# secup/ProjectUltra

Hardware: AMD Instinct MI355X
Metric: OFDM-1024 16QAM R3/4 frames decoded/sec (higher is better)
Workload: dtype f32

## Files before the change

### projectultra_amd/csrc/demod_kernel.h

```cpp
#ifndef ULTRA_DEMOD_KERNEL_H
#define ULTRA_DEMOD_KERNEL_H

#include <hip/hip_runtime.h>
#include <utility>
#include "device_types.h"
#include "pinned_math.h"
#include "phase_table.h"

namespace ultra_hip {
namespace dev {

constexpr int kWave = 64;
constexpr int kPhaseCap = 48;

__device__ __forceinline__ c32 mk(float re, float im) { c32 r; r.re = re; r.im = im; return r; }
__device__ __forceinline__ c32 cadd(c32 a, c32 b) { return mk(a.re + b.re, a.im + b.im); }
__device__ __forceinline__ c32 csub(c32 a, c32 b) { return mk(a.re - b.re, a.im - b.im); }
__device__ __forceinline__ c32 cconj(c32 a) { return mk(a.re, -a.im); }
__device__ __forceinline__ c32 cmul(c32 x, c32 y) {
    float ac = x.re * y.re, bd = x.im * y.im, ad = x.re * y.im, bc = x.im * y.re;
    return mk(ac - bd, ad + bc);
}
__device__ __forceinline__ c32 cdiv(c32 x, c32 y) {
    double a = x.re, b = x.im, c = y.re, d = y.im;
// ... 857 lines not shown
                        const float dist = dr * dr + di * di;
                        if (bits & mask) { if (dist < m1) m1 = dist; }
                        else { if (dist < m0) m0 = dist; }
                    }
                }
                out[b] = clip_llr(sf * (m1 - m0));
            }
            break;
        }
        case ULTRA_MOD_QAM64: {
            const float I = sym.re, Q = sym.im, scale = 2.0f / nv;
            const float D2 = 0.3086067f, D4 = 0.6172134f;
            out[0] = clip_llr(-scale * I);
            out[1] = clip_llr(scale * (fabsf(I) - D4));
            out[2] = clip_llr(scale * (fabsf(fabsf(I) - D4) - D2));
            out[3] = clip_llr(-scale * Q);
            out[4] = clip_llr(scale * (fabsf(Q) - D4));
            out[5] = clip_llr(scale * (fabsf(fabsf(Q) - D4) - D2));
            break;
        }
        case ULTRA_MOD_QAM256: {
            const float I = sym.re, Q = sym.im, scale = 2.0f / nv;
            const float D2 = 0.1290994f, D4 = 0.2581989f, D8 = 0.5163978f;
            out[0] = clip_llr(-scale * I);
            out[1] = clip_llr(scale * (fabsf(I) - D8));
            out[2] = clip_llr(scale * (fabsf(fabsf(I) - D8) - D4));
            out[3] = clip_llr(scale * (fabsf(fabsf(fabsf(I) - D8) - D4) - D2));
            out[4] = clip_llr(-scale * Q);
            out[5] = clip_llr(scale * (fabsf(Q) - D8));
            out[6] = clip_llr(scale * (fabsf(fabsf(Q) - D8) - D4));
            out[7] = clip_llr(scale * (fabsf(fabsf(fabsf(Q) - D8) - D4) - D2));
            break;
        }
        case ULTRA_MOD_QPSK:
        default: {
            const float scale = (-2.0f * 0.7071067811865476f) / nv;
            out[0] = clip_llr(sym.re * scale);
            out[1] = clip_llr(sym.im * scale);
            break;
        }
    }
}

__device__ __forceinline__ float slice8(float x, float d) {
    if (x < -6 * d) return -7 * d;
    if (x < -4 * d) return -5 * d;
    if (x < -2 * d) return -3 * d;
    if (x < 0) return -d;
    if (x < 2 * d) return d;
    if (x < 4 * d) return 3 * d;
    if (x < 6 * d) return 5 * d;
    return 7 * d;
}
template <int MOD>
__device__ __forceinline__ c32 hard_decision(c32 sym) {
    if (MOD == ULTRA_MOD_BPSK) return mk(sym.re > 0 ? 1.0f : -1.0f, 0.0f);
    if (MOD == ULTRA_MOD_QAM16) {
        auto slice = [](float x) { return (x < -0.4f) ? -0.9487f : (x < 0.0f) ? -0.3162f : (x < 0.4f) ? 0.3162f : 0.9487f; };
        return mk(slice(sym.re), slice(sym.im));
    }
    if (MOD == ULTRA_MOD_QAM32) {
        const float d = 0.1961161351381840f;
        const float I = (sym.re < -2 * d) ? -3 * d : (sym.re < 0) ? -d : (sym.re < 2 * d) ? d : 3 * d;
        return mk(I, slice8(sym.im, d));
    }
    if (MOD == ULTRA_MOD_QAM64) return mk(slice8(sym.re, 0.1543f), slice8(sym.im, 0.1543f));
    return mk(sym.re > 0 ? 0.7071f : -0.7071f, sym.im > 0 ? 0.7071f : -0.7071f);
}
struct AdaptiveEq { c32 w; float P; };

template <int MOD>
__device__ __forceinline__ void equalize_demap(TrackShared& sh, const DemodConst& D, const LaneConst& lc, Track& tr,
                                               c32& dprev, const c32* __restrict__ fq, float* __restrict__ llr_sym,
                                               float* dprev_abs = nullptr, const c32* tc_fixed = nullptr,
                                               const c32* received_in = nullptr, AdaptiveEq* ad = nullptr, c32* eq_out = nullptr) {
    constexpr bool kDiff = (MOD == ULTRA_MOD_DBPSK || MOD == ULTRA_MOD_DQPSK || MOD == ULTRA_MOD_D8PSK);
    constexpr int kBits = (MOD == ULTRA_MOD_DBPSK || MOD == ULTRA_MOD_BPSK) ? 1 : (MOD == ULTRA_MOD_DQPSK || MOD == ULTRA_MOD_QPSK) ? 2
                        : (MOD == ULTRA_MOD_D8PSK) ? 3 : (MOD == ULTRA_MOD_QAM16) ? 4 : (MOD == ULTRA_MOD_QAM32) ? 5
                        : (MOD == ULTRA_MOD_QAM64) ? 6 : 8;
    const int lane = threadIdx.x;
    const int nd = D.n_data;
    const bool is_data = lane < nd;
    c32 eq = mk(0.0f, 0.0f);
    float nv = 100.0f;
    if (kDiff) {
        if (is_data) {
            const c32 received = fq[lc.data_fq], h = sh.H[lc.data_slot];
            const float h_power = cnorm(h);
            const c32 tc = tc_fixed ? *tc_fixed : cexpj_bounded(timing_phase_of(lc.data_k, tr.timing, D.log2_fft));
            if (h_power > 1e-6f) {
                const c32 t = cdivf(cmul(received, cconj(h)), h_power);
                eq = cmul(cmul(t, tr.ppc), tc);
                nv = tr.noise_variance / h_power;
            } else {
                eq = cmul(cmul(received, tr.ppc), tc);
                nv = 100.0f;
            }
            nv = fmax_std(1e-6f, fmin_std(100.0f, nv));
        }
    } else {
        float h_power = 0.0f;
        if (is_data) {
            const c32 received = received_in ? *received_in : fq[lc.data_fq], h = sh.H[lc.data_slot];
            h_power = cnorm(h);
            if (ad) {
                const c32 w = ad->w;
                const float w_power = cnorm(w), denom = w_power + tr.noise_variance;
                if (denom < 1e-10f) {
                    eq = mk(0.0f, 0.0f);
                    nv = 100.0f;
                } else {
                    eq = cdivf(cmul(cconj(w), received), denom);
                    nv = tr.noise_variance / (w_power + 1e-6f);
                }
                if (D.decision_directed) {
                    const c32 ref = hard_decision<MOD>(eq);
                    const c32 err = csub(received, cmul(w, ref));
                    if (D.adaptive_eq == 2) {
                        const float lambda = D.rls_lambda, P = ad->P, ref_norm = cnorm(ref);
                        const float k = P / (lambda + P * ref_norm);
                        ad->w = cadd(w, cmul(cscale(cconj(ref), k), err));
                        const float Pn = (P - k * ref_norm * P) / lambda;
                        ad->P = fmax_std(0.001f, fmin_std(1000.0f, Pn));
                    } else {
                        ad->w = cadd(w, cmul(cscale(cconj(ref), D.lms_mu), err));
                    }
                }
            } else {
            const float mmse_denom = h_power + tr.noise_variance;
            if (mmse_denom < 1e-10f) {
                eq = mk(0.0f, 0.0f);
                nv = 100.0f;
            } else {
                eq = cdivf(cmul(cconj(h), received), mmse_denom);
                nv = tr.noise_variance / (h_power + 1e-6f);
                nv = fmax_std(1e-6f, fmin_std(100.0f, nv));
            }
            }
        }
        const float T = wave_sum_unordered(is_data ? h_power : 0.0f);
        const float thr = T * D.fade_k, lo = thr * 0.99993896484375f, hi = thr * 1.00006103515625f;
        const bool t_plain = T >= 0x1p-60f && T <= 0x1p60f;
        const bool close = is_data && !(h_power < lo) && !(h_power >= hi);
        if (__builtin_expect(t_plain && !__any(close), 1)) {
            if (is_data && h_power < lo) nv = 100.0f;
        } else {
            float avg = ordered_sum(sh.fbuf, h_power, nd);
            avg /= (float)nd;
            if (is_data && h_power < 0.1f * avg) nv = 100.0f;
        }
    }

    if (eq_out && is_data) eq_out[lane] = eq;
    if (kDiff && !tr.has_dprev) { dprev = mk(1.0f, 0.0f); if (dprev_abs) *dprev_abs = -1.0f; }
    float eq_abs = -1.0f;
    if (is_data) {
        if (kDiff) {
            eq_abs = cabs_(eq);
            const float pa = (dprev_abs && *dprev_abs >= 0.0f) ? *dprev_abs : cabs_(dprev);
            demap_carrier<MOD>(eq, dprev, nv * D.ce_margin, llr_sym + lane * kBits, eq_abs, pa);
            dprev = eq;
            if (dprev_abs) *dprev_abs = eq_abs;
        } else {
            demap_carrier<MOD>(eq, dprev, nv * D.ce_margin, llr_sym + lane * kBits);
        }
    }
    if ((MOD == ULTRA_MOD_DQPSK || MOD == ULTRA_MOD_D8PSK) && tr.snr_symbol_count >= 1) {
        bool strong = false;
        if (is_data) {
            const float a = eq_abs;
            strong = (a * a) > 0.1f;
            if (strong) sh.H[lc.data_slot] = cmul(sh.H[lc.data_slot], mk(1.0f, -0.0f));
        }
        const int valid = __popcll(__ballot(strong));
        if (valid >= 5) {
            c32 p = cmul(cscale(tr.ppc, 1.0f), mk(1.0f, -0.0f));
            const float mag = cabs_(p);
            if (mag > 0.01f) p = cdivf(p, mag);
            tr.ppc = p;
        }
    }
    if (kDiff) tr.has_dprev = 1;
    wave_sync();
}

__device__ __forceinline__ void lts_symbol(TrackShared& sh, const DemodConst& D, const LaneConst& lc, int sym,
                                           int n_train, c32& lts_acc, const c32* __restrict__ fq) {
    const int lane = threadIdx.x;
    if (lane < D.n_data && sym == n_train - 1) {
        c32 h = mk(0.0f, 0.0f);
        if (cabs_(lc.zc) > 0.01f) h = cdiv(fq[lc.data_fq], lc.zc);
        sh.H[lc.data_slot] = h;
    }
    if (lane < D.n_pilot) {
        if (sym == 0) lts_acc = mk(0.0f, 0.0f);
        if (cabs_(lc.pilot_seq) > 0.01f) lts_acc = cadd(lts_acc, cdiv_pilot(fq[lc.pilot_fq], lc.pilot_seq));
    }
    wave_sync();
}

__device__ __forceinline__ void lts_finish(TrackShared& sh, const DemodConst& D, const LaneConst& lc, Track& tr,
                                           int n_train, c32 lts_acc) {
    const int lane = threadIdx.x;
    const float inv_count = 1.0f / (float)n_train;
    if (lane < D.n_pilot) sh.H[lc.pilot_slot] = cscale(lts_acc, inv_count);
    wave_sync();
    float mag = 0.0f;
    if (lane < D.n_data) mag = cabs_(sh.H[lc.data_slot]);
    const float h_mag_avg = ordered_sum(sh.fbuf, mag, D.n_data) / (float)D.n_data;
    if (h_mag_avg > 1e-6f && tr.noise_variance > 1e-10f) {
        const float s = (h_mag_avg * h_mag_avg) / tr.noise_variance;
        tr.snr_linear = fmax_std(0.1f, fmin_std(10000.0f, s));
    }
    tr.snr_symbol_count = n_train;
    wave_sync();
}


__global__ __launch_bounds__(kWave) void init_state_kernel(const float* __restrict__ cfo_hz,
                                                           const float* __restrict__ cfo_phase, int n_frames,
                                                           float* __restrict__ state, int compact, int adaptive,
                                                           const float* __restrict__ timing = nullptr) {
    const int lane = threadIdx.x;
    for (int frame = blockIdx.x; frame < n_frames; frame += gridDim.x) {
        float* st = state + (size_t)frame * kStFloats;
        if (adaptive) {
            reinterpret_cast<c32*>(st + kStLms)[lane] = mk(1.0f, 0.0f);
            st[kStRlsP + lane] = 1.0f;
        }
        if (!compact) reinterpret_cast<c32*>(st + kStH)[lane] = mk(1.0f, 0.0f);
        if (lane < 32) reinterpret_cast<c32*>(st + kStHp)[lane] = mk(1.0f, 0.0f);
        if (lane < 16) {
            float v = 0.0f;
            const float cfo = cfo_hz ? cfo_hz[frame] : 0.0f;
            if (lane == st_cfo || lane == st_cfo_filt) v = cfo;
            else if (lane == st_cfo_phase) v = cfo_phase ? cfo_phase[frame] : 0.0f;
            else if (lane == st_noise) v = 0.1f;
            else if (lane == st_snr) v = 1.0f;
            else if (lane == st_timing) v = timing ? timing[frame] : 0.0f;
            else if (lane == st_ppc_re || lane == st_cpc_re) v = 1.0f;
            st[lane] = v;
        }
    }
}

__global__ __launch_bounds__(kWave) void resync_state_kernel(const float* __restrict__ cfo_hz, const float* __restrict__ cfo_phase,
                                                             int n_frames, float* __restrict__ state, int reset_carrier_phase) {
    const int lane = threadIdx.x;
    for (int frame = blockIdx.x; frame < n_frames; frame += gridDim.x) {
        float* st = state + (size_t)frame * kStFloats;
        if (lane < 16) {
            float v = st[lane];
            const float cfo = cfo_hz ? cfo_hz[frame] : 0.0f;
            if (lane == st_cfo || lane == st_cfo_filt) v = cfo;
            else if (lane == st_cfo_phase) v = cfo_phase ? cfo_phase[frame] : 0.0f;
            else if (lane == st_timing || lane == st_since) v = 0.0f;
            else if (lane == st_flags) {
                int flags = (int)v & ~4;
                if (reset_carrier_phase) flags &= ~1;
                v = (float)flags;
            } else if (reset_carrier_phase && lane == st_cpc_re) v = 1.0f;
            else if (reset_carrier_phase && lane == st_cpc_im) v = 0.0f;
            st[lane] = v;
        }
    }
}

__global__ __launch_bounds__(256) void train_cfo_kernel(const DemodConst* __restrict__ Dp, const c32* __restrict__ nco,
                                                        const float* __restrict__ audio, size_t frame_stride,
                                                        const unsigned* __restrict__ frame_offset, const float* __restrict__ cfo_in,
                                                        int n_frames, float* __restrict__ state) {
    const DemodConst& D = *Dp;
    const int frame = blockIdx.x * blockDim.x + threadIdx.x;
    if (frame >= n_frames || !cfo_in) return;
    const float given = cfo_in[frame];
    if (given == given) return;
    float* st = state + (size_t)frame * kStFloats;
    float cfo = 0.0f;
    if (D.n_train >= 2) {
        const float* x = audio + (size_t)frame * frame_stride + (frame_offset ? frame_offset[frame] : 0u);
        const int N = D.fft, cp = D.cp, S = D.sym_len;
        c32 P = mk(0.0f, 0.0f);
        float E1 = 0.0f, E2 = 0.0f;
        for (int i = 0; i < N; ++i) {
            const c32 o1 = nco[cp + i], o2 = nco[S + cp + i];
            const float a1 = x[cp + i], a2 = x[S + cp + i];
            const c32 z1 = mk(a1 * o1.re, a1 * -o1.im), z2 = mk(a2 * o2.re, a2 * -o2.im);
            const c32 pr = cmul(mk(z1.re, -z1.im), z2);
            P = mk(P.re + pr.re, P.im + pr.im);
            E1 += z1.re * z1.re + z1.im * z1.im;
            E2 += z2.re * z2.re + z2.im * z2.im;
        }
        const float corr = um::hypotf_(P.re, P.im) / sqrtf(E1 * E2 + 1e-10f);
        if (!(corr < 0.3f)) {
            const float phase = um::atan2f_(P.im, P.re);
            cfo = (float)((double)(phase * D.sample_rate) / ((double)2.0f * 3.14159265358979323846 * (double)S));
            const float max_cfo = D.sample_rate / (2.0f * (float)S);
            cfo = fmaxf(-max_cfo, fminf(max_cfo, cfo));
        }
    }
    st[st_cfo] = cfo; st[st_cfo_filt] = cfo; st[st_cfo_phase] = 0.0f;
}

__device__ __forceinline__ float walk_to_table(const DemodConst& D, float cfo, float phase, unsigned* __restrict__ tab) {
    tab[3] = __float_as_uint(phase);
    tab[1] = __float_as_uint(cfo);
    if (!(fabsf(cfo) > 0.01f)) { tab[0] = 0u; tab[2] = __float_as_uint(phase); return phase; }
    const float inc = (float)(((-kTwoPi) * (double)cfo) / (double)D.sample_rate);
    int covered;
    float pnext;
    const int ns = um::phase_table_walk(phase, inc, D.sym_len, kPhaseCap, &covered, &pnext,
                                        [&](int k, int start, float base, float step) {
                                            tab[4 + 3 * k] = (unsigned)start;
                                            tab[5 + 3 * k] = __float_as_uint(base);
                                            tab[6 + 3 * k] = __float_as_uint(step);
                                        });
    const unsigned bounded = (fabsf(phase) <= 4.0f && fabsf(inc) <= 1.0f) ? 0x80000000u : 0u;
    tab[0] = (unsigned)ns | ((unsigned)covered << 8) | bounded; tab[2] = __float_as_uint(pnext);
    for (int done = covered; done < D.sym_len;) {
        int c2;
        float p2;
        um::phase_table_walk(pnext, inc, D.sym_len - done, kPhaseCap, &c2, &p2, [](int, int, float, float) {});
        done += c2;
        pnext = p2;
    }
    return pnext;
}

__global__ __launch_bounds__(256) void cfo_walk_kernel(const DemodConst* __restrict__ Dp, int n_frames,
                                                       float* __restrict__ state, unsigned* __restrict__ seg_tab) {
    const DemodConst& D = *Dp;
    const int frame = blockIdx.x * blockDim.x + threadIdx.x;
    if (frame >= n_frames) return;
    float* st = state + (size_t)frame * kStFloats;
    st[st_cfo_phase] = walk_to_table(D, st[st_cfo], st[st_cfo_phase], seg_tab + (size_t)frame * kSegTabWords);
}

#ifndef UH_MIX2_WAVES
#define UH_MIX2_WAVES 3
#endif
#ifndef UH_MIX2_WAVES_NOROT
#define UH_MIX2_WAVES_NOROT 4
#endif
template <int LOG2N, bool ROT>
__global__ __launch_bounds__(Fft2Shared<LOG2N>::W * kWave) __attribute__((amdgpu_waves_per_eu(ROT ? UH_MIX2_WAVES : UH_MIX2_WAVES_NOROT, 8))) void mix_fft2_kernel(
    const DemodConst* __restrict__ Dp, const c32* __restrict__ nco, const c32* __restrict__ twiddle,
    const float* __restrict__ audio, size_t frame_stride, const unsigned* __restrict__ frame_offset, int n_frames,
    int sym, c32* __restrict__ fq, const unsigned* __restrict__ seg_tab, int n_sym_batch) {
    __shared__ Fft2Shared<LOG2N, ROT> sh;
    const DemodConst& D = *Dp;
    constexpr int P = Fft2Shared<LOG2N>::P, A = Fft2Shared<LOG2N>::A, M = Fft2Shared<LOG2N>::M, W = Fft2Shared<LOG2N>::W;
    const int h = (W == 2) ? __builtin_amdgcn_readfirstlane((int)threadIdx.x >> 6) : 0, lane = threadIdx.x & 63;
    const int rl = (int)(__brev((unsigned)lane) >> 26);
    for (int idx = threadIdx.x; idx < Fft2Shared<LOG2N>::kTwB; idx += W * kWave) {
        const int sA = 31 - __clz(idx / P + 1);
        const int k = idx - P * ((1 << sA) - 1);
        sh.twB[idx] = twiddle[k << (LOG2N - 1 - (A + sA))];
    }
    __syncthreads();
    const int total = n_frames * n_sym_batch;
    int sym_len = D.sym_len, cp = D.cp, grid_step = (int)gridDim.x;
    asm volatile("" : "+s"(sym_len), "+s"(cp), "+s"(grid_step));
    auto ds_of = [&](int w) { return (!ROT && n_sym_batch > 1) ? w / n_frames : 0; };
    auto request = [&](MixItem& it, int w) {
        const int ds = ds_of(w), f = w - ds * n_frames;
        const float* audio_sym = audio + (size_t)f * frame_stride + (frame_offset ? frame_offset[f] : 0u) + (size_t)(sym + ds) * sym_len;
        prefetch_symbol2<LOG2N, ROT>(sh, cp, h, lane, audio_sym);
        request_item(it, (ROT && seg_tab) ? seg_tab + (size_t)f * kSegTabWords : nullptr, lane);
    };
    Mix2Lane<LOG2N> lc;
    lc.w6 = twiddle[lane << (LOG2N - 7)];
    lc.w7[0] = twiddle[lane << (LOG2N - 8)]; lc.w7[1] = twiddle[(lane + 64) << (LOG2N - 8)];
    lc.w8[0] = twiddle[lane << (LOG2N - 9)]; lc.w8[1] = twiddle[(lane + 192) << (LOG2N - 9)];
    lc.w_last = (W == 2) ? twiddle[h ? (M - 64 + lane) : lane] : mk(0.0f, 0.0f);
#pragma unroll
    for (int j = 0; j < P / 2; ++j) lc.wA[j] = twiddle[j << (LOG2N - A)];
    asm volatile("" ::"v"(lc.w6.re), "v"(lc.w6.im), "v"(lc.w7[0].re), "v"(lc.w7[0].im), "v"(lc.w7[1].re), "v"(lc.w7[1].im),
                 "v"(lc.w8[0].re), "v"(lc.w8[0].im), "v"(lc.w8[1].re), "v"(lc.w8[1].im), "v"(lc.w_last.re), "v"(lc.w_last.im));
    int os_ds = -1;
    MixItem cur;
    c32 pending = mk(0.0f, 0.0f), pending_hi = mk(0.0f, 0.0f);
    const int fh = D.fq_half;
    const bool fq_mine = h ? (lane >= 64 - fh) : (lane < fh);
    const bool fq_mine_hi = W == 1 && lane >= 64 - fh;
    const int fq_slot = fq_mine ? (int)D.fq_pos[h ? fh + lane - (64 - fh) : lane] : 0;
    const int fq_slot_hi = fq_mine_hi ? (int)D.fq_pos[fh + lane - (64 - fh)] : 0;
    auto store_bins = [&](int w_item) {
        c32* row = fq + (size_t)w_item * (2 * fh);
        if (fq_mine) row[fq_slot] = pending;
        if (fq_mine_hi) row[fq_slot_hi] = pending_hi;
    };
    int w_stored = -1;
    int w = blockIdx.x;
    if (w < total) request(cur, w);
    asm volatile("s_waitcnt vmcnt(0)" ::: "memory");
    for (int par = 0; w < total; w += grid_step, par ^= 1) {
        const int ds = ds_of(w);
        if (ds != os_ds) {
            const c32* nco_sym = nco + (size_t)(sym + ds) * sym_len;
#pragma unroll
            for (int qp = 0; qp < P; ++qp) lc.os[qp] = nco_sym[cp + W * (rl + 64 * qp) + h];
            os_ds = ds;
#pragma unroll
            for (int qp = 0; qp < P; ++qp) asm volatile("" ::"v"(lc.os[qp].re), "v"(lc.os[qp].im));
            if constexpr (ROT) {
#pragma unroll
                for (int qp = 0; qp < P; ++qp) { sh.osc[h][64 * qp + lane] = lc.os[qp]; lc.os[qp] = mk(0.0f, 0.0f); }
            }
        }
        const int next = w + grid_step;
        Stamps stamps;
        c32 bin, bin_hi;
        symbol_to_freq2<LOG2N, ROT>(sh, D, h, lane, cur, lc, twiddle, bin, bin_hi, par, cp, sym_len,
                               [&]() {
                                   if (w_stored >= 0) store_bins(w_stored);
                                   if (next < total) request(cur, next);
                               }, stamps);
        pending = bin; pending_hi = bin_hi;
        w_stored = w;
        UH_STAMP(10);
        stamps.store((size_t)w * W + h, lane);
    }
    if (w_stored >= 0) store_bins(w_stored);
}

__device__ __forceinline__ void load_track(const float* __restrict__ st, Track& tr) {
    tr.freq_offset_hz = st[st_cfo]; tr.freq_offset_filtered = st[st_cfo_filt]; tr.cfo_phase = st[st_cfo_phase];
    tr.noise_variance = st[st_noise]; tr.snr_linear = st[st_snr]; tr.timing = st[st_timing];
    tr.ppc = mk(st[st_ppc_re], st[st_ppc_im]); tr.cpc = mk(st[st_cpc_re], st[st_cpc_im]);
    const int flags = (int)st[st_flags];
    tr.cpc_init = flags & 1; tr.has_prev = (flags >> 1) & 1; tr.has_dprev = (flags >> 2) & 1;
    tr.snr_symbol_count = (int)st[st_count]; tr.symbols_since_sync = (int)st[st_since];
}
__device__ __forceinline__ void store_track(float* __restrict__ st, const Track& tr) {
    st[st_cfo] = tr.freq_offset_hz; st[st_cfo_filt] = tr.freq_offset_filtered;
    st[st_noise] = tr.noise_variance; st[st_snr] = tr.snr_linear; st[st_timing] = tr.timing;
    st[st_ppc_re] = tr.ppc.re; st[st_ppc_im] = tr.ppc.im; st[st_cpc_re] = tr.cpc.re; st[st_cpc_im] = tr.cpc.im;
    st[st_flags] = (float)(tr.cpc_init | (tr.has_prev << 1) | (tr.has_dprev << 2));
    st[st_count] = (float)tr.snr_symbol_count; st[st_since] = (float)tr.symbols_since_sync;
}
__device__ __forceinline__ LaneConst lane_constants(const DemodConst& D) {
    const int lane = threadIdx.x;
    LaneConst lc;
    auto fq_of = [&](int bin) { return fq_index(D, bin); };
    const int ps = (lane < D.n_pilot) ? D.pilot_slot[lane] : 0;
    lc.pilot_slot = ps; lc.pilot_fq = fq_of(D.bin[ps]); lc.pilot_k = D.k_of[ps];
    lc.pilot_seq = (lane < D.n_pilot) ? D.pilot_seq[lane] : mk(1.0f, 0.0f);
    const int dsl = (lane < D.n_data) ? D.data_slot[lane] : 0;
    lc.data_slot = dsl; lc.data_fq = fq_of(D.bin[dsl]); lc.data_k = D.k_of[dsl];
    const int q = (lane < D.n_interp) ? lane : 0;
    lc.i_dst = D.interp_slot[q]; lc.i_lo = D.interp_lo[q]; lc.i_hi = D.interp_hi[q]; lc.i_alpha = D.interp_alpha[q];
    lc.slot_k = D.k_of[(lane < D.n_carriers) ? lane : 0];
    lc.zc = D.sync_seq[lane % D.n_carriers];
    return lc;
}

__global__ __launch_bounds__(kWave, 4) void train_kernel(const DemodConst* __restrict__ Dp, int n_frames, int sym,
                                                         float* __restrict__ state, const c32* __restrict__ fq_all) {
    __shared__ TrackShared sh;
    const DemodConst& D = *Dp;
    const int lane = threadIdx.x;
    const LaneConst lc = lane_constants(D);
    for (int frame = blockIdx.x; frame < n_frames; frame += gridDim.x) {
        float* st = state + (size_t)frame * kStFloats;
        const c32* fq = fq_all + (size_t)frame * (2 * D.fq_half);
        Track tr;
        load_track(st, tr);
        sh.H[lane] = reinterpret_cast<const c32*>(st + kStH)[lane];
        wave_sync();
        c32 lts_acc = (sym > 0 && lane < D.n_pilot) ? reinterpret_cast<const c32*>(st + kStLts)[lane] : mk(0.0f, 0.0f);
        lts_symbol(sh, D, lc, sym, D.n_train, lts_acc, fq);
        if (sym == D.n_train - 1) lts_finish(sh, D, lc, tr, D.n_train, lts_acc);
        else if (lane < D.n_pilot) reinterpret_cast<c32*>(st + kStLts)[lane] = lts_acc;
        wave_sync();
        reinterpret_cast<c32*>(st + kStH)[lane] = sh.H[lane];
        if (lane < D.n_pilot) reinterpret_cast<c32*>(st + kStHp)[lane] = sh.H[lc.pilot_slot];
        if (lane == 0) store_track(st, tr);
        wave_sync();
    }
}

template <int MOD, bool EQ = false>
__global__ __launch_bounds__(kWave, 6) void track_kernel(
    const DemodConst* __restrict__ Dp, int n_frames, int data_sym, float* __restrict__ state,
    const c32* __restrict__ fq_all, float* __restrict__ llr, size_t llr_stride, float* __restrict__ state_out,
    int n_sym_batch, int synced_loop, c32* __restrict__ eq_out = nullptr, size_t eq_stride = 0) {
    __shared__ TrackShared sh;
    const DemodConst& D = *Dp;
    const int lane = threadIdx.x;
    const LaneConst lc = lane_constants(D);
    for (int frame = blockIdx.x; frame < n_frames; frame += gridDim.x) {
        float* st = state + (size_t)frame * kStFloats;
        Track tr;
        load_track(st, tr);
        const bool presynced_loop = D.presynced && !synced_loop;
        const bool scalar_pilot_half = D.n_pilot == 0 && !presynced_loop;
        const bool compact = compact_pilot_state(D);
        if (!compact) sh.H[lane] = reinterpret_cast<const c32*>(st + kStH)[lane];
        else if (lane < D.n_pilot) sh.H[lc.pilot_slot] = reinterpret_cast<const c32*>(st + kStHp)[lane];
        c32 dprev = D.differential ? reinterpret_cast<const c32*>(st + kStDprev)[lane] : mk(1.0f, 0.0f);
        const bool adaptive = D.adaptive_eq != 0 && !D.differential;
        AdaptiveEq ad;
        ad.w = mk(1.0f, 0.0f); ad.P = 1.0f;
        if (adaptive) { ad.w = reinterpret_cast<const c32*>(st + kStLms)[lane]; ad.P = st[kStRlsP + lane]; }
        wave_sync();
        float dprev_abs = -1.0f;
        const bool tc_is_fixed = D.differential && D.n_pilot == 0 && n_sym_batch > 1;
        c32 tc0 = mk(1.0f, 0.0f);
        if (tc_is_fixed) tc0 = cexpj_bounded(timing_phase_of(lc.data_k, tr.timing, D.log2_fft));
        for (int ds = 0; ds < n_sym_batch; ++ds) {
            const c32* fq = fq_all + ((size_t)ds * n_frames + frame) * (2 * D.fq_half);
            if (scalar_pilot_half) { tr.ppc = mk(1.0f, 0.0f); tr.has_prev = 0; tr.snr_symbol_count++; }
            if (!presynced_loop || D.n_pilot != 0) {
                finish_channel_estimate(sh, D, lc, tr);
                if (adaptive && tr.snr_symbol_count - 1 < 3 && lane < D.n_data) ad.w = sh.H[lc.data_slot];
            }
            equalize_demap<MOD>(sh, D, lc, tr, dprev, fq,
                                llr + (size_t)frame * llr_stride + (size_t)(data_sym + ds) * D.llrs_per_symbol,
                                &dprev_abs, tc_is_fixed ? &tc0 : nullptr, nullptr, adaptive ? &ad : nullptr,
                                EQ ? eq_out + (size_t)frame * eq_stride + (size_t)ds * kMaxCarriers : nullptr);
            wave_sync();
        }
        if (!compact) reinterpret_cast<c32*>(st + kStH)[lane] = sh.H[lane];
        else if (lane < ((D.n_pilot + 15) & ~15))
            reinterpret_cast<c32*>(st + kStHp)[lane] = (lane < D.n_pilot) ? sh.H[lc.pilot_slot] : mk(0.0f, 0.0f);
        if (D.differential) reinterpret_cast<c32*>(st + kStDprev)[lane] = dprev;
        if (adaptive) { reinterpret_cast<c32*>(st + kStLms)[lane] = ad.w; st[kStRlsP + lane] = ad.P; }
        if (lane == 0) {
            st[st_ppc_re] = tr.ppc.re; st[st_ppc_im] = tr.ppc.im;
            st[st_flags] = (float)(tr.cpc_init | (tr.has_prev << 1) | (tr.has_dprev << 2));
            if (scalar_pilot_half) st[st_count] = (float)tr.snr_symbol_count;
            if (state_out) {
                float* so = state_out + (size_t)frame * ULTRA_HIP_STATE_FLOATS;
                so[ULTRA_HIP_STATE_FREQ_OFFSET_HZ] = tr.freq_offset_hz;
                so[ULTRA_HIP_STATE_NOISE_VARIANCE] = tr.noise_variance;
                so[ULTRA_HIP_STATE_SNR_LINEAR] = tr.snr_linear;
                so[ULTRA_HIP_STATE_TIMING_OFFSET] = tr.timing;
                so[ULTRA_HIP_STATE_CFO_PHASE] = tr.cfo_phase;
                so[ULTRA_HIP_STATE_MIXER_PHASE] = D.mixer_phase_end;
                so[ULTRA_HIP_STATE_SYMBOLS] = (float)tr.snr_symbol_count;
                so[ULTRA_HIP_STATE_RESERVED] = 0.0f;
            }
        }
        wave_sync();
    }
}

template <int MOD>
__global__ __launch_bounds__(kWave, 6) void track_diff_pair_kernel(
    const DemodConst* __restrict__ Dp, int n_frames, int data_sym, float* __restrict__ state,
    const c32* __restrict__ fq_all, float* __restrict__ llr, size_t llr_stride, float* __restrict__ state_out,
    int n_sym_batch) {
    static_assert(MOD == ULTRA_MOD_DBPSK || MOD == ULTRA_MOD_DQPSK || MOD == ULTRA_MOD_D8PSK, "differential layouts");
    constexpr int kBits = (MOD == ULTRA_MOD_DBPSK) ? 1 : (MOD == ULTRA_MOD_DQPSK) ? 2 : 3;
    const DemodConst& D = *Dp;
    const int lane = threadIdx.x, g = lane >> 5, sub = lane & 31;
    const bool is_data = sub < D.n_data;
    const int dsl = is_data ? D.data_slot[sub] : 0;
    const int data_fq = fq_index(D, D.bin[dsl]), data_k = D.k_of[dsl];
    const unsigned long long half_mask = g ? 0xffffffff00000000ull : 0x00000000ffffffffull;
    const int n_pairs = (n_frames + 1) / 2;
    for (int pair = blockIdx.x; pair < n_pairs; pair += gridDim.x) {
        const bool live = 2 * pair + g < n_frames;
        const int frame = live ? 2 * pair + g : n_frames - 1;
        float* st = state + (size_t)frame * kStFloats;
        Track tr;
        load_track(st, tr);
        c32 H = reinterpret_cast<const c32*>(st + kStH)[dsl];
        c32 dprev = reinterpret_cast<const c32*>(st + kStDprev)[sub];
        if (!tr.has_dprev) dprev = mk(1.0f, 0.0f);
        float prev_abs = cabs_(dprev);
        const c32 tc = cexpj_bounded(timing_phase_of(data_k, tr.timing, D.log2_fft));
        for (int ds = 0; ds < n_sym_batch; ++ds) {
            const c32* fq = fq_all + ((size_t)ds * n_frames + frame) * (2 * D.fq_half);
            tr.ppc = mk(1.0f, 0.0f); tr.has_prev = 0; tr.snr_symbol_count++;
            c32 eq = mk(0.0f, 0.0f);
            float nv = 100.0f;
            if (is_data) {
                const c32 received = fq[data_fq];
                const float h_power = cnorm(H);
                if (h_power > 1e-6f) {
                    const c32 t = cdivf(cmul(received, cconj(H)), h_power);
                    eq = cmul(cmul(t, tr.ppc), tc);
                    nv = tr.noise_variance / h_power;
                } else {
                    eq = cmul(cmul(received, tr.ppc), tc);
                    nv = 100.0f;
                }
                nv = fmax_std(1e-6f, fmin_std(100.0f, nv));
            }
            const float eq_abs = cabs_(eq);
            if (is_data) {
                float out[kBits];
                demap_carrier<MOD>(eq, dprev, nv * D.ce_margin, out, eq_abs, prev_abs);
                if (live) {
                    float* dst = llr + (size_t)frame * llr_stride + (size_t)(data_sym + ds) * D.llrs_per_symbol + sub * kBits;
#pragma unroll
                    for (int b = 0; b < kBits; ++b) dst[b] = out[b];
                }
                dprev = eq;
                prev_abs = eq_abs;
            }
            if ((MOD == ULTRA_MOD_DQPSK || MOD == ULTRA_MOD_D8PSK) && tr.snr_symbol_count >= 1) {
                bool strong = false;
                if (is_data) {
                    const float a = eq_abs;
                    strong = (a * a) > 0.1f;
                    if (strong) H = cmul(H, mk(1.0f, -0.0f));
                }
                const int valid = __popcll(__ballot(strong) & half_mask);
                if (valid >= 5) {
                    c32 p = cmul(cscale(tr.ppc, 1.0f), mk(1.0f, -0.0f));
                    const float mag = cabs_(p);
                    if (mag > 0.01f) p = cdivf(p, mag);
                    tr.ppc = p;
                }
            }
            tr.has_dprev = 1;
        }
        if (live && is_data) {
            reinterpret_cast<c32*>(st + kStH)[dsl] = H;
            reinterpret_cast<c32*>(st + kStDprev)[sub] = dprev;
        }
        if (live && sub == 0) {
            st[st_ppc_re] = tr.ppc.re; st[st_ppc_im] = tr.ppc.im;
            st[st_flags] = (float)(tr.cpc_init | (tr.has_prev << 1) | (tr.has_dprev << 2));
            st[st_count] = (float)tr.snr_symbol_count;
            if (state_out) {
                float* so = state_out + (size_t)frame * ULTRA_HIP_STATE_FLOATS;
                so[ULTRA_HIP_STATE_FREQ_OFFSET_HZ] = tr.freq_offset_hz;
                so[ULTRA_HIP_STATE_NOISE_VARIANCE] = tr.noise_variance;
                so[ULTRA_HIP_STATE_SNR_LINEAR] = tr.snr_linear;
                so[ULTRA_HIP_STATE_TIMING_OFFSET] = tr.timing;
                so[ULTRA_HIP_STATE_CFO_PHASE] = tr.cfo_phase;
                so[ULTRA_HIP_STATE_MIXER_PHASE] = D.mixer_phase_end;
                so[ULTRA_HIP_STATE_SYMBOLS] = (float)tr.snr_symbol_count;
                so[ULTRA_HIP_STATE_RESERVED] = 0.0f;
            }
        }
    }
}

template <int MOD>
__global__ __launch_bounds__(kWave, 6) void track_all_kernel(const DemodConst* __restrict__ Dp, int n_frames, int sym0, int n_sym_batch,
                                                             const float* __restrict__ trk_rec, const c32* __restrict__ fq_all,
                                                             float* __restrict__ llr, size_t llr_stride, float* __restrict__ state_out,
                                                             const float* __restrict__ state) {
    __shared__ TrackShared sh;
    const DemodConst& D = *Dp;
    const int lane = threadIdx.x;
    const LaneConst lc = lane_constants(D);
    const int total = n_frames * n_sym_batch;
    const int rec_floats = trk_rec_floats(D.n_pilot), rec_hp = trk_rec_hp(D.n_pilot);
    const int rec_mask = (D.n_pilot <= kTrkRecCompactPilots) ? 1 : 7;
    float nx_rec = 0.0f;
    c32 nx_hp = mk(0.0f, 0.0f), nx_fq = mk(0.0f, 0.0f);
    auto request = [&](int w) {
        const float* rec = trk_rec + (size_t)w * rec_floats;
        nx_rec = rec[lane & rec_mask];
        if (lane < D.n_pilot) nx_hp = reinterpret_cast<const c32*>(rec + rec_hp)[lane];
        if (lane < D.n_data) nx_fq = fq_all[(size_t)w * (2 * D.fq_half) + lc.data_fq];
    };
    if ((int)blockIdx.x < total) request((int)blockIdx.x);
    for (int w = blockIdx.x; w < total; w += gridDim.x) {
        const int frame = w % n_frames, ds = w / n_frames;
        Track tr;
        const float my_rec = nx_rec;
        const c32 my_hp = nx_hp, my_fq = nx_fq;
        if (w + (int)gridDim.x < total) request(w + (int)gridDim.x);
        tr.noise_variance = __int_as_float(__builtin_amdgcn_readlane(__float_as_int(my_rec), tk_noise));
        tr.timing = __int_as_float(__builtin_amdgcn_readlane(__float_as_int(my_rec), tk_timing));
        tr.ppc = mk(1.0f, 0.0f); tr.cpc = mk(1.0f, 0.0f);
        tr.cpc_init = 1; tr.has_prev = 1; tr.has_dprev = 0; tr.snr_symbol_count = 0; tr.symbols_since_sync = 0;
        if (lane < D.n_pilot) sh.H[lc.pilot_slot] = my_hp;
        c32 dprev = mk(1.0f, 0.0f);
        wave_sync();
        finish_channel_estimate(sh, D, lc, tr);
        equalize_demap<MOD>(sh, D, lc, tr, dprev, fq_all + (size_t)w * (2 * D.fq_half),
                            llr + (size_t)frame * llr_stride + (size_t)(sym0 + ds) * D.llrs_per_symbol, nullptr, nullptr, &my_fq);
        if (state_out && lane == 0 && ds == n_sym_batch - 1) {
            const float* st = state + (size_t)frame * kStFloats;
            float* so = state_out + (size_t)frame * ULTRA_HIP_STATE_FLOATS;
            so[ULTRA_HIP_STATE_FREQ_OFFSET_HZ] = st[st_cfo];
            so[ULTRA_HIP_STATE_NOISE_VARIANCE] = st[st_noise];
            so[ULTRA_HIP_STATE_SNR_LINEAR] = st[st_snr];
            so[ULTRA_HIP_STATE_TIMING_OFFSET] = st[st_timing];
            so[ULTRA_HIP_STATE_CFO_PHASE] = st[st_cfo_phase];
            so[ULTRA_HIP_STATE_MIXER_PHASE] = D.mixer_phase_end;
            so[ULTRA_HIP_STATE_SYMBOLS] = st[st_count];
            so[ULTRA_HIP_STATE_RESERVED] = 0.0f;
        }
        wave_sync();
    }
}

}
}
#endif
```

Measured before the change: 53.77 million.

## Stage CFO walk table rows in LDS and deepen track_all prefetch to two items

cfo_walk_kernel now writes the first few segment-table words for each thread into a shared-memory staging row. The wave then writes those rows to global memory cooperatively, 32 lanes per frame, so the per-thread strided scattered stores become coalesced. track_all_kernel switches from one-ahead to two-ahead software prefetch using double-buffered Ahead registers, which hides more load latency. The cost is extra LDS use and more register pressure, which can lower occupancy.

```diff
diff --git a/projectultra_amd/csrc/demod_kernel.h b/projectultra_amd/csrc/demod_kernel.h
--- a/projectultra_amd/csrc/demod_kernel.h
+++ b/projectultra_amd/csrc/demod_kernel.h
@@ -1183,21 +1183,22 @@
     st[st_cfo] = cfo; st[st_cfo_filt] = cfo; st[st_cfo_phase] = 0.0f;
 }
 
-__device__ __forceinline__ float walk_to_table(const DemodConst& D, float cfo, float phase, unsigned* __restrict__ tab) {
-    tab[3] = __float_as_uint(phase);
-    tab[1] = __float_as_uint(cfo);
-    if (!(fabsf(cfo) > 0.01f)) { tab[0] = 0u; tab[2] = __float_as_uint(phase); return phase; }
+template <class Put>
+__device__ __forceinline__ float walk_to_table(const DemodConst& D, float cfo, float phase, Put put) {
+    put(3, __float_as_uint(phase));
+    put(1, __float_as_uint(cfo));
+    if (!(fabsf(cfo) > 0.01f)) { put(0, 0u); put(2, __float_as_uint(phase)); return phase; }
     const float inc = (float)(((-kTwoPi) * (double)cfo) / (double)D.sample_rate);
     int covered;
     float pnext;
     const int ns = um::phase_table_walk(phase, inc, D.sym_len, kPhaseCap, &covered, &pnext,
                                         [&](int k, int start, float base, float step) {
-                                            tab[4 + 3 * k] = (unsigned)start;
-                                            tab[5 + 3 * k] = __float_as_uint(base);
-                                            tab[6 + 3 * k] = __float_as_uint(step);
+                                            put(4 + 3 * k, (unsigned)start);
+                                            put(5 + 3 * k, __float_as_uint(base));
+                                            put(6 + 3 * k, __float_as_uint(step));
                                         });
     const unsigned bounded = (fabsf(phase) <= 4.0f && fabsf(inc) <= 1.0f) ? 0x80000000u : 0u;
-    tab[0] = (unsigned)ns | ((unsigned)covered << 8) | bounded; tab[2] = __float_as_uint(pnext);
+    put(0, (unsigned)ns | ((unsigned)covered << 8) | bounded); put(2, __float_as_uint(pnext));
     for (int done = covered; done < D.sym_len;) {
         int c2;
         float p2;
@@ -1208,13 +1209,38 @@
     return pnext;
 }
 
+#ifndef UH_WALK_STAGE_SEGS
+#define UH_WALK_STAGE_SEGS 8
+#endif
+constexpr int kWalkStageSegs = UH_WALK_STAGE_SEGS;
+constexpr int kWalkStageWords = 4 + 3 * kWalkStageSegs;
+constexpr int kWalkStagePitch = kWalkStageWords + 1;
+static_assert(kWalkStageWords <= 32 && kWalkStageSegs <= kPhaseCap, "walk staging layout");
+
 __global__ __launch_bounds__(256) void cfo_walk_kernel(const DemodConst* __restrict__ Dp, int n_frames,
                                                        float* __restrict__ state, unsigned* __restrict__ seg_tab) {
+    __shared__ unsigned s_tab[256][kWalkStagePitch];
     const DemodConst& D = *Dp;
     const int frame = blockIdx.x * blockDim.x + threadIdx.x;
-    if (frame >= n_frames) return;
-    float* st = state + (size_t)frame * kStFloats;
-    st[st_cfo_phase] = walk_to_table(D, st[st_cfo], st[st_cfo_phase], seg_tab + (size_t)frame * kSegTabWords);
+    if (frame < n_frames) {
+        float* st = state + (size_t)frame * kStFloats;
+        unsigned* row = s_tab[threadIdx.x];
+        unsigned* tab = seg_tab + (size_t)frame * kSegTabWords;
+        st[st_cfo_phase] = walk_to_table(D, st[st_cfo], st[st_cfo_phase], [&](int j, unsigned v) {
+            if (j < kWalkStageWords) row[j] = v; else tab[j] = v;
+        });
+    }
+    wave_sync();
+    const int wbase = threadIdx.x & ~(kWave - 1), half = (threadIdx.x >> 5) & 1, j = threadIdx.x & 31;
+    for (int i = 0; i < kWave; i += 2) {
+        const int t = wbase + i + half;
+        const int f = blockIdx.x * blockDim.x + t;
+        if (f < n_frames) {
+            const int ns = (int)(s_tab[t][0] & 0xffu);
+            const int words = 4 + 3 * ((ns < kWalkStageSegs) ? ns : kWalkStageSegs);
+            if (j < words) seg_tab[(size_t)f * kSegTabWords + j] = s_tab[t][j];
+        }
+    }
 }
 
 #ifndef UH_MIX2_WAVES
@@ -1522,8 +1548,11 @@
     }
 }
 
+#ifndef UH_TRACK_ALL_WAVES
+#define UH_TRACK_ALL_WAVES 6
+#endif
 template <int MOD>
-__global__ __launch_bounds__(kWave, 6) void track_all_kernel(const DemodConst* __restrict__ Dp, int n_frames, int sym0, int n_sym_batch,
+__global__ __launch_bounds__(kWave, UH_TRACK_ALL_WAVES) void track_all_kernel(const DemodConst* __restrict__ Dp, int n_frames, int sym0, int n_sym_batch,
                                                              const float* __restrict__ trk_rec, const c32* __restrict__ fq_all,
                                                              float* __restrict__ llr, size_t llr_stride, float* __restrict__ state_out,
                                                              const float* __restrict__ state) {
@@ -1532,33 +1561,29 @@
     const int lane = threadIdx.x;
     const LaneConst lc = lane_constants(D);
     const int total = n_frames * n_sym_batch;
+    const int grid = (int)gridDim.x;
     const int rec_floats = trk_rec_floats(D.n_pilot), rec_hp = trk_rec_hp(D.n_pilot);
     const int rec_mask = (D.n_pilot <= kTrkRecCompactPilots) ? 1 : 7;
-    float nx_rec = 0.0f;
-    c32 nx_hp = mk(0.0f, 0.0f), nx_fq = mk(0.0f, 0.0f);
-    auto request = [&](int w) {
+    struct Ahead { float rec; c32 hp, fq; };
+    auto request = [&](Ahead& a, int w) {
         const float* rec = trk_rec + (size_t)w * rec_floats;
-        nx_rec = rec[lane & rec_mask];
-        if (lane < D.n_pilot) nx_hp = reinterpret_cast<const c32*>(rec + rec_hp)[lane];
-        if (lane < D.n_data) nx_fq = fq_all[(size_t)w * (2 * D.fq_half) + lc.data_fq];
+        a.rec = rec[lane & rec_mask];
+        if (lane < D.n_pilot) a.hp = reinterpret_cast<const c32*>(rec + rec_hp)[lane];
+        if (lane < D.n_data) a.fq = fq_all[(size_t)w * (2 * D.fq_half) + lc.data_fq];
     };
-    if ((int)blockIdx.x < total) request((int)blockIdx.x);
-    for (int w = blockIdx.x; w < total; w += gridDim.x) {
+    auto item = [&](int w, const Ahead& my) {
         const int frame = w % n_frames, ds = w / n_frames;
         Track tr;
-        const float my_rec = nx_rec;
-        const c32 my_hp = nx_hp, my_fq = nx_fq;
-        if (w + (int)gridDim.x < total) request(w + (int)gridDim.x);
-        tr.noise_variance = __int_as_float(__builtin_amdgcn_readlane(__float_as_int(my_rec), tk_noise));
-        tr.timing = __int_as_float(__builtin_amdgcn_readlane(__float_as_int(my_rec), tk_timing));
+        tr.noise_variance = __int_as_float(__builtin_amdgcn_readlane(__float_as_int(my.rec), tk_noise));
+        tr.timing = __int_as_float(__builtin_amdgcn_readlane(__float_as_int(my.rec), tk_timing));
         tr.ppc = mk(1.0f, 0.0f); tr.cpc = mk(1.0f, 0.0f);
         tr.cpc_init = 1; tr.has_prev = 1; tr.has_dprev = 0; tr.snr_symbol_count = 0; tr.symbols_since_sync = 0;
-        if (lane < D.n_pilot) sh.H[lc.pilot_slot] = my_hp;
+        if (lane < D.n_pilot) sh.H[lc.pilot_slot] = my.hp;
         c32 dprev = mk(1.0f, 0.0f);
         wave_sync();
         finish_channel_estimate(sh, D, lc, tr);
         equalize_demap<MOD>(sh, D, lc, tr, dprev, fq_all + (size_t)w * (2 * D.fq_half),
-                            llr + (size_t)frame * llr_stride + (size_t)(sym0 + ds) * D.llrs_per_symbol, nullptr, nullptr, &my_fq);
+                            llr + (size_t)frame * llr_stride + (size_t)(sym0 + ds) * D.llrs_per_symbol, nullptr, nullptr, &my.fq);
         if (state_out && lane == 0 && ds == n_sym_batch - 1) {
             const float* st = state + (size_t)frame * kStFloats;
             float* so = state_out + (size_t)frame * ULTRA_HIP_STATE_FLOATS;
@@ -1572,6 +1597,19 @@
             so[ULTRA_HIP_STATE_RESERVED] = 0.0f;
         }
         wave_sync();
+    };
+    Ahead a = {0.0f, mk(0.0f, 0.0f), mk(0.0f, 0.0f)}, b = a;
+    const int w0 = blockIdx.x;
+    if (w0 < total) request(a, w0);
+    if (w0 + grid < total) request(b, w0 + grid);
+    for (int w = w0; w < total; w += 2 * grid) {
+        const Ahead my_a = a;
+        if (w + 2 * grid < total) request(a, w + 2 * grid);
+        item(w, my_a);
+        if (w + grid >= total) break;
+        const Ahead my_b = b;
+        if (w + 3 * grid < total) request(b, w + 3 * grid);
+        item(w + grid, my_b);
     }
 }
 
```

New measurement: 54.26 million, median of 6. No clear change (+0.9%).
